# Spimp/sparc_ldpc

Hardware: AMD Instinct MI355X
Metric: decoded codewords/sec (T AMP iters) at L=512,M=512; achieved HBM GB/s vs roofline (higher is better)
Workload: dtype f32; 1 GPU; BASELINE configs[1]: L=512 M=512 R=1 P=4, T=64, single codeword; L=512, M=512, n=4608, T=64, backend=hadamard, precision=fp32, early_stop=False, parallelism=reps sharded over 1 GPU(s)

## Files before the change

### include/sparc_amp.h

```cpp
#ifndef SPARC_AMP_H
#define SPARC_AMP_H

#include <stdint.h>

#ifdef __cplusplus
extern "C" {
#endif

typedef struct sa_ctx sa_ctx;

enum {
  SA_OK = 0,
  SA_ERR_ARG = -1,
  SA_ERR_HIP = -2,
  SA_ERR_NOMEM = -3,
  SA_ERR_ORDERING = -4,
  SA_ERR_UNSUPPORTED = -5,
  SA_ERR_NO_DEVICE = -6
};

enum {
  SA_BACKEND_HADAMARD = 0,
  SA_BACKEND_DENSE = 1,
  SA_BACKEND_HOST = 2,
  SA_BACKEND_MATRIX = 3
};

enum { SA_PREC_F32 = 0, SA_PREC_F64 = 1 };

enum {
  SA_FLAG_NO_EARLY_STOP = 1,
  SA_FLAG_BETA0 = 0x100,
  SA_PTR_DEVICE = 0x200
};

int sa_create(sa_ctx** out, int L, int M, int n, const uint32_t* ordering,
              int backend, int precision, int device);

enum {
  SA_PLAN_DEFAULT = 0,
  SA_PLAN_SEC3 = 1 << 0,
  SA_PLAN_NO_SEC3 = 1 << 1,
  SA_PLAN_ROW16 = 1 << 2,
  SA_PLAN_NO_ROW16 = 1 << 3,
  SA_PLAN_NO_PT = 1 << 4,
  SA_PLAN_ZIL = 1 << 5,
  SA_PLAN_NO_ZIL = 1 << 6,
  SA_PLAN_WB8 = 1 << 7,
  SA_PLAN_WB16 = 1 << 8,
  SA_PLAN_NO_BANKS = 1 << 9,
  SA_PLAN_EAGER = 1 << 10,
  SA_PLAN_ONE_PASS = 1 << 11,
  SA_PLAN_NO_LANES = 1 << 12,
  SA_PLAN_ALL = (1 << 13) - 1
};
int sa_create_ex(sa_ctx** out, int L, int M, int n, const uint32_t* ordering,
                 int backend, int precision, int device, int plan);

int sa_create_matrix(sa_ctx** out, int L, int M, int n, const double* A,
                     int precision, int device);

int sa_create_matrix_random(sa_ctx** out, int L, int M, int n, uint64_t seed, double scale,
                            int precision, int device);

int sa_subset(const sa_ctx* parent, const int64_t* sections, int Ls, sa_ctx** out);

int sa_create_twin(sa_ctx* src, sa_ctx** out);

void sa_destroy(sa_ctx* ctx);

int sa_Ab(sa_ctx* ctx, int B, const double* beta, double* out);

int sa_Az(sa_ctx* ctx, int B, const double* z, double* out);

int sa_amp(sa_ctx* ctx, int B, const double* y, const double* Pl, int T,
           const double* beta0, double* beta_out, int* iters_out, int flags);

int sa_reserve(sa_ctx* ctx, int B, int T);
int sa_stage(sa_ctx* ctx, int B, const double* y, const double* Pl, const double* beta0);
int sa_stage_power_batch(sa_ctx* ctx, int B, const double* Pl);
int sa_run(sa_ctx* ctx, int B, int T, int flags);
int sa_wait(sa_ctx* ctx);
int sa_fetch(sa_ctx* ctx, int B, double* beta_out, int* iters_out);
int sa_fetch_z(sa_ctx* ctx, int B, double* z_out);
int sa_fetch_y(sa_ctx* ctx, int B, double* y_out);
double sa_run_event_ms(sa_ctx* ctx);

// ... 23 lines not shown
                   int32_t* idx_out);

int sa_threshold(sa_ctx* ctx, int B, int l0, int ns, const double* app, int flags, double threshold,
                 int32_t* idx_out);

int sa_cancel(sa_ctx* ctx, int B, const int32_t* idx, sa_ctx* dst);

int sa_cancel_scaled(sa_ctx* ctx, int B, const int32_t* idx, double scale, sa_ctx* dst);

int sa_host_init(sa_ctx* ctx, int B, int T, const double* y, const double* Pl, const double* beta0,
                 const double* ab0);
int sa_host_tau(sa_ctx* ctx, int B, int t, int flags, int* stopped);
int sa_host_eta(sa_ctx* ctx, int B, int t, int flags, const double* az);
int sa_host_residual(sa_ctx* ctx, int B, int t, int flags, const double* ab);

int sa_draw_reps(const uint32_t* seeds, int count, int L, int M, int n, double sigma, int32_t* idx_out,
                 double* noise_out, int threads);
int sa_mc_stage(sa_ctx* ctx, int nreps, const int32_t* idx, const double* noise);
int sa_mc_run(sa_ctx* ctx, int B, int T, int flags, int32_t* dec_out, int32_t* iters_out, int32_t* errs_out,
              double* ms_out);
int sa_mc_draw(sa_ctx* ctx, int nreps, const uint32_t* seeds, const double* sigma, double* ms_out);
int sa_mc_fetch_draws(sa_ctx* ctx, int nreps, int32_t* idx_out, double* noise_out);
int sa_make_ordering(int L, int M, int n, uint32_t seed, uint32_t* out);

typedef enum sa_sec_path {
  SA_SEC_K_SEC = 0,
  SA_SEC_K_SEC2 = 1,
  SA_SEC_K_SECB = 2,
  SA_SEC_DENSE = 3,
  SA_SEC_K_SEC4 = 4,
  SA_SEC_K_SEC43 = 5,
  SA_SEC_DENSE_I8 = 6,
  SA_SEC_MATRIX = 7,
  SA_SEC_K_SECG = 8
} sa_sec_path;
typedef enum sa_row_kernel {
  SA_ROW_K_ROW = 0,
  SA_ROW_K_ROW2 = 1,
  SA_ROW_K_ROWV16 = 2,
  SA_ROW_K_ROWV8 = 3,
  SA_ROW_K_ROW2_16 = 4,
  SA_ROW_K_ROWC = 5
} sa_row_kernel;
int sa_plan(sa_ctx* ctx, int B, int64_t* out8);
int sa_plan_batched(sa_ctx* ctx, int B, int64_t* out4);
int sa_info(const sa_ctx* ctx, int64_t* out8);
int sa_device_count(void);
const char* sa_last_error(void);
const char* sa_version(void);

#ifdef __cplusplus
}
#endif
#endif
```

### sparc_ldpc_amd/_lib.py

```python
from __future__ import annotations

import ctypes as ct
import os

import numpy as np

LIB_NAME = "libsparc_amp.so"
LIB_PATH = os.environ.get("SPARC_AMP_LIB") or os.path.join(os.path.dirname(os.path.abspath(__file__)), LIB_NAME)

SA_OK = 0
SA_ERR_ARG = -1
SA_ERR_HIP = -2
SA_ERR_NOMEM = -3
SA_ERR_ORDERING = -4
SA_ERR_UNSUPPORTED = -5
SA_ERR_NO_DEVICE = -6

SA_BACKEND_HADAMARD = 0
SA_BACKEND_DENSE = 1
SA_BACKEND_HOST = 2
SA_BACKEND_MATRIX = 3
SA_PREC_F32 = 0
SA_PREC_F64 = 1
SA_FLAG_NO_EARLY_STOP = 1
SA_FLAG_BETA0 = 0x100
SA_PTR_DEVICE = 0x200

SA_PLAN = {
    "SEC3": 1 << 0, "NO_SEC3": 1 << 1, "ROW16": 1 << 2, "NO_ROW16": 1 << 3, "NO_PT": 1 << 4,
    "ZIL": 1 << 5, "NO_ZIL": 1 << 6, "WB8": 1 << 7, "WB16": 1 << 8, "NO_BANKS": 1 << 9, "EAGER": 1 << 10,
    "ONE_PASS": 1 << 11, "NO_LANES": 1 << 12,
}


def plan_bits(plan) -> int:
    if plan is None:
        return 0
    if isinstance(plan, int):
        return plan
    if isinstance(plan, str):
        plan = [plan]
    bits = 0
    for name in plan:
        key = name.upper()
        if key not in SA_PLAN:
            raise ValueError(f"unknown plan option {name!r}; known: {sorted(SA_PLAN)}")
        bits |= SA_PLAN[key]
    return bits

EXPORTS = (
    "sa_create", "sa_create_ex", "sa_create_matrix", "sa_create_matrix_random", "sa_subset", "sa_create_twin", "sa_destroy", "sa_Ab", "sa_Az", "sa_amp",
    "sa_reserve", "sa_stage", "sa_stage_power_batch", "sa_run", "sa_wait", "sa_fetch", "sa_fetch_z", "sa_fetch_y", "sa_run_event_ms",
    "sa_profile", "sa_profile_rep", "sa_profile_dispatch", "sa_profile_kinds", "sa_decide",
    "sa_decide_async", "sa_decide_collect", "sa_info", "sa_device_count", "sa_last_error", "sa_version",
    "sa_encode", "sa_stage_onehot", "sa_llr", "sa_soft_beta0", "sa_hard_cancel",
    "sa_threshold", "sa_cancel", "sa_plan", "sa_plan_batched", "sa_stage_onehot_scaled", "sa_cancel_scaled",
    "sa_host_init", "sa_host_tau", "sa_host_eta", "sa_host_residual",
    "sa_draw_reps", "sa_mc_stage", "sa_mc_run", "sa_make_ordering", "sa_mc_draw", "sa_mc_fetch_draws",
)

_P = ct.c_void_p
_I = ct.c_int
_D = ct.POINTER(ct.c_double)
_SIG = {
# ... 119 lines not shown
```

### sparc_ldpc_amd/csrc/sa_host.h

```cpp
#pragma once
#include "sa_common.h"

namespace sa {

struct Prof {
  std::vector<std::tuple<int, hipEvent_t, hipEvent_t>> ev;
  int rep = 1;
  bool dispatch = false;
  int kind = 0;
  int begin(hipStream_t s, int k) {
    kind = k;
    if (dispatch) return 0;
    hipEvent_t a = nullptr, b = nullptr;
    if (add(&a, &b)) return -1;
    return hipEventRecord(a, s) == hipSuccess ? 0 : -1;
  }
  void end(hipStream_t s) {
    if (!dispatch) (void)hipEventRecord(std::get<2>(ev.back()), s);
  }
  int add(hipEvent_t* a, hipEvent_t* b) {
    *a = *b = nullptr;
    if (hipEventCreate(a) != hipSuccess || hipEventCreate(b) != hipSuccess) return -1;
    ev.emplace_back(kind, *a, *b);
    return 0;
// ... 25 lines not shown
  unsigned long long y_ver = 0;
  bool y_read = false;
};

struct sa_ctx {
  sa::Prof* prof = nullptr;
  enum { kLanes = 2 };
  sa_lane lane[kLanes];
  int cur = 0;
  sa_lane& at() { return lane[cur]; }
  const sa_lane& at() const { return lane[cur]; }
  bool lanes_on = false;
  unsigned long long y_ver = 0;
  int y_lane = 0;
  std::vector<double> h_Pl;
  std::vector<double> h_Plb;
  int L = 0, M = 0, n = 0, w = 0, nhi = 0, backend = 0, prec = 0, device = 0;
  int plan = 0;
  bool pow2 = true;
  int Mu = 0, dead = 0;
  int G = 0, NZ = 0, E = 1;
  int n_cus = 256;
  int Gb = 0, CB = 0;
  int WB = 8;
  int gpx = 1 << 20;
  size_t secb_lds = 0;
  int RS = 1, KS = 1, Gd = 0;
  size_t lda = 0;
  size_t sec_lds = 0;
  int G2 = 0;
  int G3 = 0;
  bool sec3 = false;
  size_t sec3_lds = 0;
  uint32_t* d_fwd3 = nullptr;
  bool pt_on = false;
  bool sec4 = false;
  size_t sec4_lds = 0;
  int NZ16 = 0;
  int NZh = 0;
  bool row16 = false;
  int NZ4 = 0, NZ2 = 0;
  bool zil_last = false;
  size_t sec2_lds = 0;
  std::vector<uint32_t> ordering;
  uint16_t* d_inv = nullptr;
  bool big = false;
  uint32_t* d_inv32 = nullptr;
  uint16_t* d_invb = nullptr;
  uint16_t* d_fwdb = nullptr;
  uint16_t* d_invl = nullptr;
  uint32_t* d_hs = nullptr;
  bool borrowed = false;
  bool invb_done = false;
  uint16_t* d_fwd = nullptr;
  uint32_t* d_fwd2 = nullptr;
  void* d_A = nullptr;
  int8_t *d_A8 = nullptr, *d_AT8 = nullptr, *d_zq = nullptr, *d_bq = nullptr;
  double *d_zsc = nullptr, *d_bsc0 = nullptr, *d_bfix = nullptr;
  long long np8 = 0, LMp8 = 0;
  int Bp8 = 0;
  long long np = 0, nk = 0, LMy = 0;
  void *d_AT = nullptr, *d_xz = nullptr, *d_xb = nullptr;
  int fg_cap = 0;
  double cmax = 0;
  int Bcap = 0, Tcap = 0;
  void *d_out = nullptr, *d_c = nullptr, *d_azp = nullptr;
// ... 62 lines not shown
  return SA_OK;
}

constexpr int kI8MinB = 4;
constexpr int kI8MaxS = 16;
constexpr int kFMinB = 4;
constexpr int kFMaxS = 16;

inline size_t rsz(const sa_ctx* c) { return c->prec == SA_PREC_F64 ? 8 : 4; }

inline bool is_dense(const sa_ctx* c) { return c->backend == SA_BACKEND_DENSE || c->backend == SA_BACKEND_MATRIX; }
inline bool use_i8(const sa_ctx* c, int B) { return c->backend == SA_BACKEND_DENSE && B >= kI8MinB; }
inline bool use_fgemm(const sa_ctx* c, int B) { return c->backend == SA_BACKEND_MATRIX && B >= kFMinB; }
inline bool use_batched(const sa_ctx* c, int B) { return c->CB > 0 && B >= 4; }

inline bool zil_for(const sa_ctx* c, int B) {
  const bool on = (c->plan & SA_PLAN_NO_ZIL) ? false : true;
  return on && c->backend == SA_BACKEND_HADAMARD && use_batched(c, B) && c->CB * (int)rsz(c) == 16;
}

int dense_parts(const sa_ctx* c, int B);

struct Plan {
  sa_sec_path sec = SA_SEC_K_SEC;
  sa_row_kernel row = SA_ROW_K_ROW;
  int nz = 0;
  int G = 0, Gb = 0;
  int pt = 0;
  int rs = 1;
  int CB = 1;
  bool zil = false;
  bool dense() const { return sec == SA_SEC_DENSE || sec == SA_SEC_DENSE_I8 || sec == SA_SEC_MATRIX; }
  bool batched() const { return sec == SA_SEC_K_SECB; }
  bool multiwave() const { return sec == SA_SEC_K_SEC2 || sec == SA_SEC_K_SEC4 || sec == SA_SEC_K_SEC43; }
  bool row_sets_iters() const { return row == SA_ROW_K_ROW2 || row == SA_ROW_K_ROW2_16; }
  bool it_row() const { return !dense() && !batched() && row_sets_iters(); }
  bool bzero() const { return sec == SA_SEC_K_SEC4 || sec == SA_SEC_K_SEC43; }
};

inline Plan plan_for(const sa_ctx* c, int B) {
  Plan p;
  const bool f32 = c->prec == SA_PREC_F32;
  p.zil = zil_for(c, B);
  if (p.zil) {
    p.row = SA_ROW_K_ROWC; p.nz = c->NZ2;
  } else if ((long long)B * c->NZ < 4LL * c->n_cus) {
    if (c->row16 && B == 1) { p.row = SA_ROW_K_ROW2_16; p.nz = c->NZh; }
    else { p.row = SA_ROW_K_ROW2; p.nz = c->NZ16; }
  } else if (c->n % (f32 ? 4 : 2) == 0 && (long long)B * (f32 ? c->NZ4 : c->NZ2) >= 2LL * c->n_cus) {
    p.row = SA_ROW_K_ROWV16; p.nz = f32 ? c->NZ4 : c->NZ2;
  } else if (f32 && c->n % 2 == 0 && (long long)B * c->NZ2 >= 2LL * c->n_cus) {
    p.row = SA_ROW_K_ROWV8; p.nz = c->NZ2;
  } else {
    p.row = SA_ROW_K_ROW; p.nz = c->NZ;
  }
  const int wgs = c->G * B;
  p.rs = std::min(4, std::max(1, (c->n_cus + wgs - 1) / wgs));
  if (is_dense(c)) {
    p.sec = use_i8(c, B) ? SA_SEC_DENSE_I8 : (use_fgemm(c, B) ? SA_SEC_MATRIX : SA_SEC_DENSE);
    p.G = dense_parts(c, B);
    p.Gb = c->Gd;
  } else if (use_batched(c, B)) {
    p.sec = SA_SEC_K_SECB;
    p.G = p.Gb = c->Gb;
    p.CB = c->CB;
  } else if (c->backend == SA_BACKEND_HADAMARD && c->G2 > 0 && c->G2 * B * 2 >= c->n_cus) {
    p.sec = c->sec3 ? SA_SEC_K_SEC43 : (c->sec4 ? SA_SEC_K_SEC4 : SA_SEC_K_SEC2);
    p.G = p.Gb = c->sec3 ? c->G3 : c->G2;
    if (p.sec != SA_SEC_K_SEC2 && p.row_sets_iters() && c->pt_on) p.pt = p.row == SA_ROW_K_ROW2_16 ? 16 : kRow2Rows;
  } else {
    p.sec = c->big ? SA_SEC_K_SECG : SA_SEC_K_SEC;
    p.G = p.Gb = c->G;
  }
  return p;
}

template <typename real>
SecArgs<real> sec_args(sa_ctx* c, const Plan& p, int mode, int t, int early_stop, const int* tb = nullptr) {
  SecArgs<real> a;
  const sa_lane& ln = c->at();
  a.inv = c->d_inv; a.inv32 = c->d_inv32; a.invb = c->d_invb; a.invl = c->d_invl; a.hs = c->d_hs;
  a.fwd = (const ushort4*)c->d_fwd;
  a.fwdb = (const ushort4*)c->d_fwdb; a.fwd2 = c->d_fwd2; a.fwd3 = c->d_fwd3; a.c = (const real*)c->d_c;
  a.z = (const real*)ln.d_z; a.beta = (real*)ln.d_beta; a.beta_out = (real*)ln.d_beta; a.out = (real*)c->d_out;
  a.abp = (real*)ln.d_abp; a.bbp = (real*)ln.d_bbp; a.zzp = (const real*)ln.d_zzp;
  a.tau = (real*)ln.d_tau; a.iters = ln.d_iters;
  a.L = c->L; a.M = c->M; a.n = c->n; a.w = c->w; a.nhi = c->nhi; a.G = c->G; a.NZ = p.nz;
  a.T1 = c->Tcap + 1; a.t = t; a.mode = mode; a.early_stop = early_stop;
  a.RS = 1;
  a.pt = 0;
  a.B = 0; a.NC = 0; a.zil = 0; a.gpx = 1 << 20;
  a.cst = c->pb_on ? c->L : 0;
  if (c->pb_on) a.c = (const real*)c->d_cb;
  a.sqrt_n = (real)std::sqrt((double)c->n);
  a.tb = tb;
  a.dead = c->dead;
  a.bzero = 0;
  return a;
}

template <typename real>
// ... 107 lines not shown
```

### sparc_ldpc_amd/csrc/sa_row.hip

```cpp
#include "sa_host.h"

namespace sa {

template <typename real, int kRowWaves>
__global__ void __launch_bounds__(kRowWaves * 64) k_row(RowArgs<real> a) {
  __shared__ real red[kRowWaves][kRowsPerBlk];
  const int b = blockIdx.y, tid = threadIdx.x, lane = tid & 63, wv = tid >> 6;
  const int r = blockIdx.x * kRowsPerBlk + lane;
  const int n = a.n;
  real tau = 1, last = 0;
  if (a.mode == ROW_AMP) {
    tau = ld_vmem(a.tau + (size_t)b * a.T1 + a.t);
    last = a.t > 0 ? ld_vmem(a.tau + (size_t)b * a.T1 + a.t - 1) : (real)0;
  }
  const size_t o = (size_t)b * n + (r < n ? r : 0);
  real yv = 0, zv = 0, Pv = 0, bbv[2] = {0, 0};
  if (wv == 0) {
    yv = a.y[o];
    if (a.mode == ROW_AMP) {
      zv = a.z[o];
      Pv = ld_vmem(a.Pb + (size_t)b * a.Pbst);
      const real* bp = a.bbp + (size_t)b * a.Gb;
      bbv[0] = lane < a.Gb ? bp[lane] : (real)0;
      bbv[1] = lane + 64 < a.Gb ? bp[lane + 64] : (real)0;
// ... 272 lines not shown
  const int rl = tid & (R - 1), pg = tid / R;
  const int r = blockIdx.x * R + rl;
  real tau = 1, last = 0;
  if (mode == ROW_AMP) {
    tau = ld_vmem(tau_p + (size_t)b * T1 + t);
    last = t > 0 ? ld_vmem(tau_p + (size_t)b * T1 + t - 1) : (real)0;
  }
  const size_t o = (size_t)b * n + (r < n ? r : 0);
  real yv = 0, zv = 0, Pv = 0, bbv[4] = {0, 0, 0, 0};
  if (tid < 64) {
    yv = y_p[o];
    if (mode == ROW_AMP) {
      zv = zin_p[o];
      Pv = ld_vmem(Pb_p + (size_t)b * Pbst);
      const real* bp = bbp_p + (size_t)b * Gb;
#pragma unroll
      for (int q = 0; q < 4; ++q) bbv[q] = tid + 64 * q < Gb ? bp[tid + 64 * q] : (real)0;
    }
  }
  if (mode != ROW_INIT0) {
    const size_t gs = pt ? (size_t)R : (size_t)n;
    const real* p = pt ? abp_p + (size_t)b * G * ((size_t)NZ * R) + (size_t)blockIdx.x * G * R + rl
                       : abp_p + (size_t)b * G * n + (r < n ? r : 0);
    real acc = 0;
    constexpr int U = 256 / NG;
    if (pt && (R == 16 || sizeof(real) == 4) && G == NG * U) {
      const real* pb = abp_p + (size_t)b * G * ((size_t)NZ * R) + (size_t)blockIdx.x * G * R;
      real tt[U];
#pragma unroll
      for (int u = 0; u < U; ++u)
        tt[u] = ld_off(pb, (unsigned)(((pg + NG * u) * R + rl) * (int)sizeof(real)));
#pragma unroll
      for (int u = 0; u < U; ++u) acc += tt[u];
    } else
    for (int g0 = pg; g0 < G; g0 += NG * U) {
      real tt[U];
#pragma unroll
      for (int u = 0; u < U; ++u) {
        const int g = g0 + NG * u;
        tt[u] = p[(size_t)(g < G ? g : pg) * gs];
      }
#pragma unroll
      for (int u = 0; u < U; ++u)
        if (g0 + NG * u < G) acc += tt[u];
    }
    red[pg][rl] = acc;
  }
  if (mode == ROW_AMP && es && tau == last) return;
  const real tau2 = tau * tau;
  __syncthreads();
  if (tid >= 64) return;
  if (itset != 0 && blockIdx.x == 0 && tid == 0) iters_p[b] = itset;
  real ons = 0;
  if (mode == ROW_AMP) {
    real bb;
    if (Gb <= 256) {
      real sacc = 0;
#pragma unroll
      for (int q = 0; q < 4; ++q) sacc += bbv[q];
      bb = wave_sum(sacc);
    } else {
      bb = wave_sum_parts(bbp_p + (size_t)b * Gb, Gb);
    }
    ons = Pv - bb / (real)n;
  }
  real zn = 0;
// ... 90 lines not shown
```

### sparc_ldpc_amd/csrc/sa_sec.hip

```cpp
#include "sa_host.h"

namespace sa {



template <typename real, int E>
__global__ void __launch_bounds__(256) k_sec(SecArgs<real> a) {
  STAMP(0);
  extern __shared__ __attribute__((aligned(16))) unsigned char smem[];
  constexpr int KH = E >= 16 ? 2 : (E >= 8 ? 16 : 16);
  constexpr int NQ = (E + 3) / 4;
  constexpr int KR = 8;
  int g, rsi;
  if (a.RS > 1 && (a.G & 7) == 0) {
    const int j = blockIdx.x, u = j >> 3;
    rsi = u % a.RS;
    g = (u / a.RS) * 8 + (j & 7);
  } else {
    g = blockIdx.x / a.RS;
    rsi = blockIdx.x % a.RS;
  }
  const int b = blockIdx.y;
  const int rows_per = (a.n + a.RS - 1) / a.RS;
  const int rb0 = rsi * rows_per, rb1 = min(a.n, rb0 + rows_per);
// ... 450 lines not shown
  for (int i = 0; i < EQ; ++i) xs[q * QS + i * 64 + lane] = v[i];
  __syncthreads();
#pragma unroll
  for (int i = 0; i < EQ; ++i) {
    real x[QW];
#pragma unroll
    for (int j = 0; j < QW; ++j) x[j] = xs[j * QS + i * 64 + lane];
#pragma unroll
    for (int k = 0, span = 1; span < QW; ++k, span <<= 1)
#pragma unroll
      for (int j = 0; j < QW; j += 2 * span) x[j] = ((q >> k) & 1) ? x[j] - x[j + span] : x[j] + x[j + span];
    v[i] = x[0];
  }
  __syncthreads();
}

template <typename real, int QW, bool MAX>
__device__ __forceinline__ real combine_q(const real* red, int w0, int f) {
  real x[QW];
#pragma unroll
  for (int j = 0; j < QW; ++j) x[j] = red[(w0 + j) * 4 + f];
#pragma unroll
  for (int span = 1; span < QW; span <<= 1)
#pragma unroll
    for (int j = 0; j < QW; j += 2 * span) {
      if constexpr (MAX) x[j] = x[j] > x[j + span] ? x[j] : x[j + span];
      else x[j] = x[j] + x[j + span];
    }
  return x[0];
}

template <typename real, int EQ, int QW, int SPW = 2>
__device__ __forceinline__ void secq_body(const SecArgs<real>& a) {
  static_assert(SPW == 2 || SPW == 3, "sections per workgroup");
  STAMP(0);
  extern __shared__ __attribute__((aligned(16))) unsigned char smem[];
  constexpr int NT = SPW * QW * 64;
  constexpr int KH = EQ >= 8 ? 4 : (SPW == 3 ? 8 : 16);
  constexpr int NQ = (EQ + 3) / 4;
  constexpr int KR = ((SPW == 3 ? 8448 : 4608) + NT - 1) / NT;
  const int g = blockIdx.x, b = blockIdx.y;
  const int tid = threadIdx.x, lane = tid & 63, wv = tid >> 6;
  const int sidx = wv / QW, q = wv % QW;
  const int M = a.M, n = a.n, Mq = M / QW;
  const size_t LM = (size_t)a.L * M;
  const int l = g * SPW + sidx;
  const bool have = l < a.L;
  const int lc = have ? l : a.L - 1;
  const int eoff = q * Mq;

  real* zs = reinterpret_cast<real*>(smem);
  const int zslots = ((n + 1) * (int)sizeof(real) + 15) / 16 * 16 / (int)sizeof(real);
  real* ts = zs + zslots;
  real* xb = ts + SPW * M;
  real* red = xb + SPW * M;

  real v[EQ];
  real bprev[EQ];
  const real* bl = a.beta + (size_t)b * LM + (size_t)lc * M + eoff;
  real* blo = a.beta_out + (size_t)b * LM + (size_t)lc * M + eoff;
  const uint16_t* ibase = a.inv + (size_t)g * SPW * a.w;
  const unsigned ioff = (unsigned)((lc - g * SPW) * a.w + eoff);
  const uint32_t* fw = (SPW == 2 ? a.fwd2 : a.fwd3) + (size_t)g * n;
  ushort4 tb[KH][NQ];
  uint32_t f[KR];

  const real* zb = a.z + (size_t)b * n;
  ZStage<real, NT> zst;
  const real* zzb = a.zzp + (size_t)b * a.NZ;
  ZZParts<real, 5> zz;
  const bool dma = stage_z_dma<real, NT>(zb, zs, n, tid);
  if (!dma) zst.issue(zb, n, tid);
  zz.issue(zzb, a.NZ, lane);
  const real last = a.t > 0 ? ld_vmem(a.tau + (size_t)b * a.T1 + a.t - 1) : (real)0;
  load_buckets_off<EQ, KH>(ibase, ioff, 0, a.nhi, M, lane, tb);
  load_section<real, EQ>(bl, bprev, lane, Mq);
  const real cl = ld_vmem(a.c + (size_t)b * a.cst + lc);
  const real tau = zz.tau(zzb, a.NZ, n);
  if (a.bzero) {
#pragma unroll
    for (int i = 0; i < EQ; ++i) bprev[i] = 0;
  }
  const bool stop = a.early_stop && (tau == last);
  if (g == 0 && tid == 0) {
    a.tau[(size_t)b * a.T1 + a.t] = tau;
    if (stop && a.iters[b] < 0) a.iters[b] = a.t;
  }
  if (stop) {
    if (dma) asm volatile("s_waitcnt vmcnt(0)" ::: "memory");
    if (a.bzero && have) {
      store_section<real, EQ>(a.beta + (size_t)b * LM + (size_t)lc * M + eoff, bprev, lane, Mq);
    }
    return;
  }
  const real tau2 = tau * tau;
  const real inv_sn = (real)1 / a.sqrt_n;
  const real kk = cl / tau2;
  STAMP(1);
  if (!dma) zst.store(zs, zb, n, tid);
  else finish_z_dma<real>(zb, zs, n, tid);
  __syncthreads();
  STAMP(2);
#ifdef SA_STAMPS
  asm volatile("s_waitcnt vmcnt(0)" ::: "memory");
  STAMP(10);
#endif
#pragma unroll
  for (int i = 0; i < EQ; ++i) v[i] = 0;
  for (int h0 = 0; h0 < a.nhi; h0 += KH) {
    ushort4 tn[KH][NQ];
    const bool more = h0 + KH < a.nhi;
    if (more) load_buckets_off<EQ, KH>(ibase, ioff, h0 + KH, a.nhi, M, lane, tn);
    gather_buckets<real, EQ, KH>(zs, h0, a.nhi, tb, v);
    if (more) {
#pragma unroll
      for (int hh = 0; hh < KH; ++hh)
#pragma unroll
        for (int j = 0; j < NQ; ++j) tb[hh][j] = tn[hh][j];
    }
  }
  real* xs = xb + sidx * M;
#pragma unroll
  for (int u = 0; u < KR; ++u) {
    const int r = u * NT + tid;
    f[u] = ld_off(fw, (unsigned)(r < n ? r : 0) * 4u);
  }
  STAMP(3);
  fwht_wave<real, EQ>(v, lane, 64);
  topq_stage<real, EQ, QW>(v, xs, lane, q);
  STAMP(4);


  real mx = neg_inf<real>();
#pragma unroll
  for (int i = 0; i < EQ; ++i) {
    v[i] = fma(v[i], inv_sn, bprev[i]) * kk;
    mx = v[i] > mx ? v[i] : mx;
  }
  mx = wave_max(mx);
  if (lane == 0) red[wv * 4] = mx;
  __syncthreads();
  const int w0 = wv & ~(QW - 1);
  mx = combine_q<real, QW, true>(red, w0, 0);
  real S = 0, S2 = 0;
#pragma unroll
  for (int i = 0; i < EQ; ++i) {
    v[i] = dexp<real>(v[i] - mx);
    S += v[i];
    S2 += v[i] * v[i];
  }
  wave_sum2(S, S2);
  if (lane == 0) {
    red[wv * 4 + 1] = S;
    red[wv * 4 + 2] = S2;
  }
  __syncthreads();
  S = combine_q<real, QW, false>(red, w0, 1);
  S2 = combine_q<real, QW, false>(red, w0, 2);
  const real scale = cl * rcp_fast(S);
#pragma unroll
  for (int i = 0; i < EQ; ++i) v[i] = have ? v[i] * scale : (real)0;
  if (have) store_section<real, EQ>(blo, v, lane, Mq);
  const real bb = have ? S2 * scale * scale : (real)0;

  STAMP(5);
  fwht_wave<real, EQ>(v, lane, 64);
  topq_stage<real, EQ, QW>(v, xs, lane, q);
  STAMP(6);
  {
    real* tl = ts + sidx * M + eoff;
#pragma unroll
    for (int i = 0; i < EQ; ++i) tl[elem_index<EQ>(lane, i)] = v[i];
  }
  if (lane == 0) red[wv * 4 + 3] = bb;
  __syncthreads();
  STAMP(7);
  if (tid == 0) {
    real bsum = red[0 * 4 + 3] + red[QW * 4 + 3];
    if constexpr (SPW == 3) bsum += red[2 * QW * 4 + 3];
    a.bbp[(size_t)b * a.G + g] = bsum;
  }
  real* abp = a.abp + ((size_t)b * a.G + g) * n;
  const int psh = a.pt == 16 ? 4 : 5;
  const size_t npad = (size_t)((n + (1 << psh) - 1) >> psh) << psh;
  real* abq = a.abp + (size_t)b * a.G * npad + ((size_t)g << psh);
  real* const sbase = a.pt ? abq : abp;
  const int sh = a.pt ? psh : 31;
  const size_t gstride = (size_t)a.G << sh;
  const int smask = (int)((1u << sh) - 1u);
  static_assert(NT % 32 == 0, "a pass of rows is a whole number of row blocks");
  const size_t ustep = sh < 31 ? (size_t)(NT >> sh) * gstride : (size_t)NT;
  for (int r0 = 0; r0 < n; r0 += NT * KR) {
    if (r0 > 0) {
#pragma unroll
      for (int u = 0; u < KR; ++u) {
        const int r = r0 + u * NT + tid;
        f[u] = fw[r < n ? r : 0];
      }
    }
    real* const pbase = sbase + (size_t)((r0 + tid) >> sh) * gstride + ((r0 + tid) & smask);
    auto row = [&](int u, int r) {
      real t;
      if constexpr (SPW == 2) {
        const uint32_t e = f[u];
        const real v0 = ts[e & 0x7fffu];
        const real v1 = ts[M + ((e >> 16) & 0x7fffu)];
        t = (e & 0x8000u) ? -v0 : v0;
        t += (e & 0x80000000u) ? -v1 : v1;
      } else {
        const uint32_t e = f[u];
        const real v0 = ts[e & 0x1ffu];
        const real v1 = ts[M + ((e >> 10) & 0x1ffu)];
        const real v2 = ts[2 * M + ((e >> 20) & 0x1ffu)];
        t = (e & 0x200u) ? -v0 : v0;
        t += (e & 0x80000u) ? -v1 : v1;
        t += (e & 0x20000000u) ? -v2 : v2;
      }
      if constexpr (SPW == 3) st_part(pbase + u * ustep, t);
      else st_part(&sbase[(size_t)(r >> sh) * gstride + (r & smask)], t);
    };
    if (r0 + NT * KR <= n) {
#pragma unroll
      for (int u = 0; u < KR; ++u) row(u, r0 + u * NT + tid);
    } else {
#pragma unroll
      for (int u = 0; u < KR; ++u) {
        const int r = r0 + u * NT + tid;
        if (r < n) row(u, r);
      }
    }
  }
#ifdef SA_STAMPS
  STAMP(8);
  asm volatile("s_waitcnt vmcnt(0)" ::: "memory");
  STAMP(9);
#endif
}

template <typename real, int E4>
__global__ void __launch_bounds__(512) k_sec4(SecArgs<real> a) { secq_body<real, E4, 4, 2>(a); }
template <typename real, int E4>
__global__ void __launch_bounds__(768) k_sec43(SecArgs<real> a) { secq_body<real, E4, 4, 3>(a); }

template <typename real, int E>
void launch_sec_e(sa_ctx* c, const Plan& p, int B, SecArgs<real> a) {
  a.RS = p.rs;
  dim3 grid(c->G * a.RS, B);
  if (c->prof) c->prof->begin(c->at().stream, K_SEC);
  if (c->big)
    plaunch(c, k_secg<real, E>, grid, 256, c->sec_lds, a);
  else
    plaunch(c, k_sec<real, E>, grid, 256, c->sec_lds, a);
  if (c->prof) c->prof->end(c->at().stream);
}

template <typename real>
int launch_sec2(sa_ctx* c, const Plan& p, int B, int t, int es, void* bin, void* bout, int bzero) {
  SecArgs<real> a = sec_args<real>(c, p, SEC_AMP, t, es);
  a.pt = p.pt;
  if (bzero && !p.bzero()) return fail(SA_ERR_UNSUPPORTED, "k_sec2 reads its previous estimate");
  a.bzero = bzero;
  a.beta = (real*)bin;
  a.beta_out = (real*)bout;
  a.G = p.G;
  dim3 grid(a.G, B);
  if (c->prof) c->prof->begin(c->at().stream, K_SEC);
  switch (p.sec) {
    case SA_SEC_K_SEC43:
      switch (c->M / 256) {
        case 1: plaunch(c, k_sec43<real, 1>, grid, 768, c->sec3_lds, a); break;
        case 2: plaunch(c, k_sec43<real, 2>, grid, 768, c->sec3_lds, a); break;
        default: return fail(SA_ERR_UNSUPPORTED, "k_sec43: M");
      }
      break;
    case SA_SEC_K_SEC4:
      switch (c->M / 256) {
        case 1: plaunch(c, k_sec4<real, 1>, grid, 512, c->sec4_lds, a); break;
        case 2: plaunch(c, k_sec4<real, 2>, grid, 512, c->sec4_lds, a); break;
        case 4: plaunch(c, k_sec4<real, 4>, grid, 512, c->sec4_lds, a); break;
        case 8: plaunch(c, k_sec4<real, 8>, grid, 512, c->sec4_lds, a); break;
        case 16: plaunch(c, k_sec4<real, 16>, grid, 512, c->sec4_lds, a); break;
        default: return fail(SA_ERR_UNSUPPORTED, "k_sec4: M");
      }
      break;
    case SA_SEC_K_SEC2:
      switch (c->M / 128) {
        case 1: plaunch(c, k_sec2<real, 1>, grid, 256, c->sec2_lds, a); break;
        case 2: plaunch(c, k_sec2<real, 2>, grid, 256, c->sec2_lds, a); break;
        case 4: plaunch(c, k_sec2<real, 4>, grid, 256, c->sec2_lds, a); break;
        case 8: plaunch(c, k_sec2<real, 8>, grid, 256, c->sec2_lds, a); break;
        case 16: plaunch(c, k_sec2<real, 16>, grid, 256, c->sec2_lds, a); break;
        case 32: plaunch(c, k_sec2<real, 32>, grid, 256, c->sec2_lds, a); break;
        default: return fail(SA_ERR_UNSUPPORTED, "k_sec2: M");
      }
      break;
    default: return fail(SA_ERR_ARG, "launch_sec2: the plan runs no multi-wave section kernel");
  }
  if (c->prof) c->prof->end(c->at().stream);
  HIP_TRY(hipGetLastError());
  return SA_OK;
}

template <typename real>
int launch_sec(sa_ctx* c, const Plan& p, int B, int mode, int t, int es, void* bin, void* bout) {
  SecArgs<real> a = sec_args<real>(c, p, mode, t, es);
  if (bin) a.beta = (real*)bin;
  if (bout) a.beta_out = (real*)bout;
  switch (c->E) {
    case 1: launch_sec_e<real, 1>(c, p, B, a); break;
    case 2: launch_sec_e<real, 2>(c, p, B, a); break;
    case 4: launch_sec_e<real, 4>(c, p, B, a); break;
    case 8: launch_sec_e<real, 8>(c, p, B, a); break;
    case 16: launch_sec_e<real, 16>(c, p, B, a); break;
    case 32: launch_sec_e<real, 32>(c, p, B, a); break;
    case 64: launch_sec_e<real, 64>(c, p, B, a); break;
    default: return fail(SA_ERR_UNSUPPORTED, "bad E");
  }
  HIP_TRY(hipGetLastError());
  return SA_OK;
}

template int launch_sec<float>(sa_ctx*, const Plan&, int, int, int, int, void*, void*);
template int launch_sec<double>(sa_ctx*, const Plan&, int, int, int, int, void*, void*);
template int launch_sec2<float>(sa_ctx*, const Plan&, int, int, int, void*, void*, int);
template int launch_sec2<double>(sa_ctx*, const Plan&, int, int, int, void*, void*, int);

template <typename real>
static hipError_t sec_lds_attrs_t() {
  const int mx = 160 * 1024;
  hipError_t e = hipSuccess;
#define SA_A(F) if (e == hipSuccess) e = hipFuncSetAttribute((const void*)F, hipFuncAttributeMaxDynamicSharedMemorySize, mx);
  SA_A((k_sec<real, 1>)) SA_A((k_sec<real, 2>)) SA_A((k_sec<real, 4>)) SA_A((k_sec<real, 8>))
  SA_A((k_sec<real, 16>)) SA_A((k_sec<real, 32>)) SA_A((k_sec<real, 64>))
  SA_A((k_secg<real, 1>)) SA_A((k_secg<real, 2>)) SA_A((k_secg<real, 4>)) SA_A((k_secg<real, 8>))
  SA_A((k_secg<real, 16>)) SA_A((k_secg<real, 32>)) SA_A((k_secg<real, 64>))
  SA_A((k_sec2<real, 1>)) SA_A((k_sec2<real, 2>)) SA_A((k_sec2<real, 4>)) SA_A((k_sec2<real, 8>))
  SA_A((k_sec2<real, 16>)) SA_A((k_sec2<real, 32>))
  SA_A((k_sec4<real, 1>)) SA_A((k_sec4<real, 2>)) SA_A((k_sec4<real, 4>)) SA_A((k_sec4<real, 8>))
  SA_A((k_sec4<real, 16>))
  SA_A((k_sec43<real, 1>)) SA_A((k_sec43<real, 2>))
#undef SA_A
  return e;
}

hipError_t sec_lds_attrs() {
  hipError_t e = sec_lds_attrs_t<float>();
  return e == hipSuccess ? sec_lds_attrs_t<double>() : e;
}

#ifdef SA_STAMPS
hipError_t stamps_add_sec(unsigned long long* out) {
  unsigned long long s[16 * 16];
  hipError_t e = hipMemcpyFromSymbol(s, HIP_SYMBOL(g_stamps), sizeof(s));
  for (int i = 0; i < 16 * 16; ++i) out[i] += s[i];
  return e;
}
#endif

}
```

### sparc_ldpc_amd/csrc/sparc_amp.hip

```cpp

#define SA_VERSION "sparc_amp 0.4 gfx950"

#include "sa_host.h"

namespace sa {

thread_local std::string g_err;

int fail(int code, const std::string& msg) {
  g_err = msg;
  return code;
}

template <typename src_t, typename dst_t>
__global__ void k_convert(const src_t* s, dst_t* d, size_t N) {
  for (size_t i = blockIdx.x * (size_t)blockDim.x + threadIdx.x; i < N;
       i += (size_t)gridDim.x * blockDim.x)
    d[i] = (dst_t)s[i];
}

__global__ void k_fill32(uint32_t* p, uint32_t v, size_t nw) {
  for (size_t i = blockIdx.x * (size_t)blockDim.x + threadIdx.x; i < nw; i += (size_t)gridDim.x * blockDim.x)
    p[i] = v;
}
// ... 972 lines not shown
    const auto c8 = nob ? std::pair<int, size_t>{0, 0} : cb_for(kWB);
    const auto c16 = nob ? std::pair<int, size_t>{0, 0} : cb_for(kWB16);
    const bool w16 = (plan & SA_PLAN_WB16) ? true
                     : (plan & SA_PLAN_WB8) ? false
                                            : c16.first >= c8.first;
    c->WB = w16 && c16.first > 0 ? kWB16 : kWB;
    c->CB = c->WB == kWB16 ? c16.first : c8.first;
    c->secb_lds = c->WB == kWB16 ? c16.second : c8.second;
    c->Gb = (L + c->WB - 1) / c->WB;
    const size_t per_group = (size_t)c->WB * ((size_t)c->w + (size_t)n) * 2;
    const int gx = c->Gb / 8 > 0 ? c->Gb / 8 : 1;
    const int fit = (int)std::max<size_t>(1, kSecbL2 / per_group);
    int npass = (gx + fit - 1) / fit;
    c->gpx = (gx + npass - 1) / npass;
    if (plan & SA_PLAN_ONE_PASS) c->gpx = 1 << 20;
  }
  {
    hipDeviceProp_t prop;
    if (hipGetDeviceProperties(&prop, device) == hipSuccess && prop.multiProcessorCount > 0)
      c->n_cus = prop.multiProcessorCount;
  }
  c->Gd = (L + 3) / 4;
  {
    const size_t need3 = (((size_t)(n + 1) * s + 15) / 16 * 16) + 6 * (size_t)M * s + 48 * s;
    const int G3 = (L + 2) / 3;
    const bool fits = c->sec4 && backend == SA_BACKEND_HADAMARD && M <= 512 && need3 <= 160 * 1024;
    const bool over = c->G2 > c->n_cus || (s == 8 && c->G2 == c->n_cus);
    const bool want = (plan & SA_PLAN_SEC3) ? true : (plan & SA_PLAN_NO_SEC3) ? false : (over && G3 <= c->n_cus);
    if (fits && want) {
      c->sec3 = true;
      c->G3 = G3;
      c->sec3_lds = need3;
    }
  }
  if (lane_open(c->lane[0]) != SA_OK) {
    delete c;
    return fail(SA_ERR_HIP, "stream/event creation failed");
  }
  int rc = SA_OK;
  if (backend == SA_BACKEND_DENSE) {
    c->RS = 8;
    c->KS = 8;
    rc = build_tables(c);
    if (!rc) rc = build_dense(c);
  } else if (backend == SA_BACKEND_HOST) {
    c->lda = (size_t)L * M;
  } else if (backend == SA_BACKEND_MATRIX) {
    c->RS = 8;
    c->KS = 8;
    rc = matrix_init(c);
  } else if (share) {
    c->d_inv = share->d_inv; c->d_inv32 = share->d_inv32; c->d_invb = share->d_invb;
    c->d_fwdb = share->d_fwdb; c->d_fwd = share->d_fwd; c->d_fwd2 = share->d_fwd2; c->d_fwd3 = share->d_fwd3;
    c->d_invl = share->d_invl; c->d_hs = share->d_hs;
    c->invb_done = share->invb_done;
    c->borrowed = true;
  } else {
    rc = build_tables(c);
  }
  if (!rc) rc = dev_alloc(c, &c->d_c, (size_t)L * s);
  if (!rc) rc = dev_alloc(c, (void**)&c->d_cd, (size_t)L * 8);
  if (!rc) rc = dev_alloc(c, &c->d_P1, s);
  if (rc) {
    sa_destroy(c);
    return rc;
  }
// ... 420 lines not shown
```

### sparc_ldpc_amd/operators.py

```python
from __future__ import annotations

import hashlib
import os
from collections import OrderedDict

import numpy as np

from . import _lib
from ._lib import as_f64, check, dptr

__all__ = [
    "SparcOperator", "AbOp", "AzOp", "HostOperatorLoop", "make_ordering", "sub_fht", "block_sub_fht",
    "sparc_transforms", "sparc_transforms_shorter", "dense_transforms", "gaussian_transforms", "default_device",
]

_BACKENDS = {"hadamard": _lib.SA_BACKEND_HADAMARD, "dense": _lib.SA_BACKEND_DENSE}
_PRECS = {"fp32": _lib.SA_PREC_F32, "fp64": _lib.SA_PREC_F64}

DEFAULT_BACKEND = os.environ.get("SPARC_AMP_BACKEND", "hadamard")
DEFAULT_PRECISION = os.environ.get("SPARC_AMP_PRECISION", "fp32")


def default_device() -> int:
    lib = _lib.load()
# ... 202 lines not shown
        check(self._lib.sa_wait(self._ctx))

    def last_run_ms(self) -> float:
        return float(self._lib.sa_run_event_ms(self._ctx))

    KERNEL_KINDS = ("k_sec", "k_row", "k_dense_az", "k_dense_den", "k_dense_ab", "k_i8_quant")

    def profile(self, B, T, early_stop=True, beta0=False, rep=1):
        flags = (0 if early_stop else _lib.SA_FLAG_NO_EARLY_STOP) | (_lib.SA_FLAG_BETA0 if beta0 else 0)
        nk = len(self.KERNEL_KINDS)
        if int(self._lib.sa_profile_kinds()) != nk:
            raise _lib.SparcAmpError(_lib.SA_ERR_UNSUPPORTED, f"libsparc_amp profiles {self._lib.sa_profile_kinds()} kernel kinds, "
                                f"this module knows {nk}: rebuild the library")
        out = np.zeros(2 * nk + 1)
        if rep == 0:
            check(self._lib.sa_profile_dispatch(self._ctx, int(B), int(T), flags, dptr(out)))
        else:
            check(self._lib.sa_profile_rep(self._ctx, int(B), int(T), flags, int(rep), dptr(out)))
        kinds = {k: (float(out[2 * i]), int(out[2 * i + 1])) for i, k in enumerate(self.KERNEL_KINDS)}
        return kinds, float(out[2 * nk])

    def fetch(self, B):
        out = np.empty((B, self.L * self.M))
        iters = np.empty(B, dtype=np.int32)
        check(self._lib.sa_fetch(self._ctx, B, dptr(out), iters.ctypes.data_as(_lib.ct.POINTER(_lib.ct.c_int))))
        return out, iters

    def iters(self, B):
        it = np.empty(B, dtype=np.int32)
        check(self._lib.sa_fetch(self._ctx, B, None, it.ctypes.data_as(_lib.ct.POINTER(_lib.ct.c_int))))
        return it

    SECTION_KERNELS = ("k_sec", "k_sec2", "k_secb", "dense", "k_sec4", "k_sec43", "dense_mfma", "matrix_mfma",
                       "k_secg")
    ROW_KERNELS = ("k_row", "k_row2", "k_rowv16B", "k_rowv8B", "k_row2_16", "k_rowc")

    def fetch_z(self, B):
        z = np.empty((B, self.n))
        check(self._lib.sa_fetch_z(self._ctx, int(B), z.ctypes.data_as(_lib.ct.POINTER(_lib.ct.c_double))))
        return z

    def fetch_y(self, B):
        y = np.empty((B, self.n))
        check(self._lib.sa_fetch_y(self._ctx, int(B), dptr(y)))
        return y

    def plan(self, B):
        o = np.zeros(8, dtype=np.int64)
        check(self._lib.sa_plan(self._ctx, int(B), o.ctypes.data_as(_lib.ct.POINTER(_lib.ct.c_int64))))
        return dict(section_kernel=self.SECTION_KERNELS[int(o[0])], partials=int(o[1]), row_splits=int(o[2]),
                    codewords_per_wg=int(o[3]), zz_partials=int(o[4]), w=int(o[5]),
                    row_kernel=self.ROW_KERNELS[int(o[6])], cus=int(o[7]))

    def mc_supported(self, B):
        if self.backend != "hadamard" or not 4 <= int(B) <= 1024:
            return False
        p = self.plan(B)
        return p["section_kernel"] == "k_secb" and p["row_kernel"] == "k_rowc"

    def mc_stage(self, idx, noise):
        idx = np.ascontiguousarray(idx, dtype=np.int32)
        R = idx.shape[0]
        assert idx.shape == (R, self.L), "idx must be (R, L)"
        noise = as_f64(noise)
        assert noise.size == R * self.n, "noise must be (R, n)"
        check(self._lib.sa_mc_stage(self._ctx, R, idx.ctypes.data_as(_lib.ct.POINTER(_lib.ct.c_int32)), dptr(noise)))
        self._mc_reps = R
# ... 316 lines not shown
```

Before: 2275 codewords/s.

## Add opt-in four-sections-per-workgroup section kernel and adjust row16 default

```diff
diff --git a/include/sparc_amp.h b/include/sparc_amp.h
--- a/include/sparc_amp.h
+++ b/include/sparc_amp.h
@@ -52,7 +52,9 @@
   SA_PLAN_EAGER = 1 << 10,
   SA_PLAN_ONE_PASS = 1 << 11,
   SA_PLAN_NO_LANES = 1 << 12,
-  SA_PLAN_ALL = (1 << 13) - 1
+  SA_PLAN_SEC4Q = 1 << 13,
+  SA_PLAN_NO_SEC4Q = 1 << 14,
+  SA_PLAN_ALL = (1 << 15) - 1
 };
 int sa_create_ex(sa_ctx** out, int L, int M, int n, const uint32_t* ordering,
                  int backend, int precision, int device, int plan);
@@ -142,7 +144,8 @@
   SA_SEC_K_SEC43 = 5,
   SA_SEC_DENSE_I8 = 6,
   SA_SEC_MATRIX = 7,
-  SA_SEC_K_SECG = 8
+  SA_SEC_K_SECG = 8,
+  SA_SEC_K_SEC44 = 9
 } sa_sec_path;
 typedef enum sa_row_kernel {
   SA_ROW_K_ROW = 0,
diff --git a/sparc_ldpc_amd/_lib.py b/sparc_ldpc_amd/_lib.py
--- a/sparc_ldpc_amd/_lib.py
+++ b/sparc_ldpc_amd/_lib.py
@@ -29,7 +29,7 @@
 SA_PLAN = {
     "SEC3": 1 << 0, "NO_SEC3": 1 << 1, "ROW16": 1 << 2, "NO_ROW16": 1 << 3, "NO_PT": 1 << 4,
     "ZIL": 1 << 5, "NO_ZIL": 1 << 6, "WB8": 1 << 7, "WB16": 1 << 8, "NO_BANKS": 1 << 9, "EAGER": 1 << 10,
-    "ONE_PASS": 1 << 11, "NO_LANES": 1 << 12,
+    "ONE_PASS": 1 << 11, "NO_LANES": 1 << 12, "SEC4Q": 1 << 13, "NO_SEC4Q": 1 << 14,
 }
 
 
diff --git a/sparc_ldpc_amd/csrc/sa_host.h b/sparc_ldpc_amd/csrc/sa_host.h
--- a/sparc_ldpc_amd/csrc/sa_host.h
+++ b/sparc_ldpc_amd/csrc/sa_host.h
@@ -81,6 +81,9 @@
   int G3 = 0;
   bool sec3 = false;
   size_t sec3_lds = 0;
+  int G4 = 0;
+  bool sec4q = false;
+  size_t sec4q_lds = 0;
   uint32_t* d_fwd3 = nullptr;
   bool pt_on = false;
   bool sec4 = false;
@@ -209,10 +212,12 @@
   bool zil = false;
   bool dense() const { return sec == SA_SEC_DENSE || sec == SA_SEC_DENSE_I8 || sec == SA_SEC_MATRIX; }
   bool batched() const { return sec == SA_SEC_K_SECB; }
-  bool multiwave() const { return sec == SA_SEC_K_SEC2 || sec == SA_SEC_K_SEC4 || sec == SA_SEC_K_SEC43; }
+  bool multiwave() const {
+    return sec == SA_SEC_K_SEC2 || sec == SA_SEC_K_SEC4 || sec == SA_SEC_K_SEC43 || sec == SA_SEC_K_SEC44;
+  }
   bool row_sets_iters() const { return row == SA_ROW_K_ROW2 || row == SA_ROW_K_ROW2_16; }
   bool it_row() const { return !dense() && !batched() && row_sets_iters(); }
-  bool bzero() const { return sec == SA_SEC_K_SEC4 || sec == SA_SEC_K_SEC43; }
+  bool bzero() const { return sec == SA_SEC_K_SEC4 || sec == SA_SEC_K_SEC43 || sec == SA_SEC_K_SEC44; }
 };
 
 inline Plan plan_for(const sa_ctx* c, int B) {
@@ -242,8 +247,8 @@
     p.G = p.Gb = c->Gb;
     p.CB = c->CB;
   } else if (c->backend == SA_BACKEND_HADAMARD && c->G2 > 0 && c->G2 * B * 2 >= c->n_cus) {
-    p.sec = c->sec3 ? SA_SEC_K_SEC43 : (c->sec4 ? SA_SEC_K_SEC4 : SA_SEC_K_SEC2);
-    p.G = p.Gb = c->sec3 ? c->G3 : c->G2;
+    p.sec = c->sec3 ? SA_SEC_K_SEC43 : (c->sec4q ? SA_SEC_K_SEC44 : (c->sec4 ? SA_SEC_K_SEC4 : SA_SEC_K_SEC2));
+    p.G = p.Gb = c->sec3 ? c->G3 : (c->sec4q ? c->G4 : c->G2);
     if (p.sec != SA_SEC_K_SEC2 && p.row_sets_iters() && c->pt_on) p.pt = p.row == SA_ROW_K_ROW2_16 ? 16 : kRow2Rows;
   } else {
     p.sec = c->big ? SA_SEC_K_SECG : SA_SEC_K_SEC;
diff --git a/sparc_ldpc_amd/csrc/sa_row.hip b/sparc_ldpc_amd/csrc/sa_row.hip
--- a/sparc_ldpc_amd/csrc/sa_row.hip
+++ b/sparc_ldpc_amd/csrc/sa_row.hip
@@ -328,6 +328,15 @@
         tt[u] = ld_off(pb, (unsigned)(((pg + NG * u) * R + rl) * (int)sizeof(real)));
 #pragma unroll
       for (int u = 0; u < U; ++u) acc += tt[u];
+    } else if (pt && (R == 16 || sizeof(real) == 4) && G == NG * (U / 2)) {
+      constexpr int UH = U / 2;
+      const real* pb = abp_p + (size_t)b * G * ((size_t)NZ * R) + (size_t)blockIdx.x * G * R;
+      real tt[UH];
+#pragma unroll
+      for (int u = 0; u < UH; ++u)
+        tt[u] = ld_off(pb, (unsigned)(((pg + NG * u) * R + rl) * (int)sizeof(real)));
+#pragma unroll
+      for (int u = 0; u < UH; ++u) acc += tt[u];
     } else
     for (int g0 = pg; g0 < G; g0 += NG * U) {
       real tt[U];
diff --git a/sparc_ldpc_amd/csrc/sa_sec.hip b/sparc_ldpc_amd/csrc/sa_sec.hip
--- a/sparc_ldpc_amd/csrc/sa_sec.hip
+++ b/sparc_ldpc_amd/csrc/sa_sec.hip
@@ -506,13 +506,14 @@
 
 template <typename real, int EQ, int QW, int SPW = 2>
 __device__ __forceinline__ void secq_body(const SecArgs<real>& a) {
-  static_assert(SPW == 2 || SPW == 3, "sections per workgroup");
+  static_assert(SPW == 2 || SPW == 3 || SPW == 4, "sections per workgroup");
   STAMP(0);
   extern __shared__ __attribute__((aligned(16))) unsigned char smem[];
   constexpr int NT = SPW * QW * 64;
-  constexpr int KH = EQ >= 8 ? 4 : (SPW == 3 ? 8 : 16);
+  constexpr int KH = EQ >= 8 ? 4 : ((SPW == 3 || (SPW == 4 && sizeof(real) == 8)) ? 8 : 16);
   constexpr int NQ = (EQ + 3) / 4;
   constexpr int KR = ((SPW == 3 ? 8448 : 4608) + NT - 1) / NT;
+  constexpr int FW = SPW == 4 ? 2 : 1;
   const int g = blockIdx.x, b = blockIdx.y;
   const int tid = threadIdx.x, lane = tid & 63, wv = tid >> 6;
   const int sidx = wv / QW, q = wv % QW;
@@ -535,9 +536,10 @@
   real* blo = a.beta_out + (size_t)b * LM + (size_t)lc * M + eoff;
   const uint16_t* ibase = a.inv + (size_t)g * SPW * a.w;
   const unsigned ioff = (unsigned)((lc - g * SPW) * a.w + eoff);
-  const uint32_t* fw = (SPW == 2 ? a.fwd2 : a.fwd3) + (size_t)g * n;
+  const uint32_t* fw = (SPW == 3 ? a.fwd3 : a.fwd2) + (size_t)(SPW == 4 ? 2 * g : g) * n;
+  const uint32_t* fw1 = a.fwd2 + (size_t)(2 * g + 1 < (a.L + 1) / 2 ? 2 * g + 1 : 2 * g) * n;
   ushort4 tb[KH][NQ];
-  uint32_t f[KR];
+  uint32_t f[KR][FW];
 
   const real* zb = a.z + (size_t)b * n;
   ZStage<real, NT> zst;
@@ -597,7 +599,8 @@
 #pragma unroll
   for (int u = 0; u < KR; ++u) {
     const int r = u * NT + tid;
-    f[u] = ld_off(fw, (unsigned)(r < n ? r : 0) * 4u);
+    f[u][0] = ld_off(fw, (unsigned)(r < n ? r : 0) * 4u);
+    if constexpr (SPW == 4) f[u][1] = ld_off(fw1, (unsigned)(r < n ? r : 0) * 4u);
   }
   STAMP(3);
   fwht_wave<real, EQ>(v, lane, 64);
@@ -651,7 +654,8 @@
   STAMP(7);
   if (tid == 0) {
     real bsum = red[0 * 4 + 3] + red[QW * 4 + 3];
-    if constexpr (SPW == 3) bsum += red[2 * QW * 4 + 3];
+    if constexpr (SPW >= 3) bsum += red[2 * QW * 4 + 3];
+    if constexpr (SPW == 4) bsum += red[3 * QW * 4 + 3];
     a.bbp[(size_t)b * a.G + g] = bsum;
   }
   real* abp = a.abp + ((size_t)b * a.G + g) * n;
@@ -669,20 +673,32 @@
 #pragma unroll
       for (int u = 0; u < KR; ++u) {
         const int r = r0 + u * NT + tid;
-        f[u] = fw[r < n ? r : 0];
+        f[u][0] = fw[r < n ? r : 0];
+        if constexpr (SPW == 4) f[u][1] = fw1[r < n ? r : 0];
       }
     }
     real* const pbase = sbase + (size_t)((r0 + tid) >> sh) * gstride + ((r0 + tid) & smask);
     auto row = [&](int u, int r) {
       real t;
       if constexpr (SPW == 2) {
-        const uint32_t e = f[u];
+        const uint32_t e = f[u][0];
         const real v0 = ts[e & 0x7fffu];
         const real v1 = ts[M + ((e >> 16) & 0x7fffu)];
         t = (e & 0x8000u) ? -v0 : v0;
         t += (e & 0x80000000u) ? -v1 : v1;
+      } else if constexpr (SPW == 4) {
+        const uint32_t e = f[u][0], e1 = f[u][1];
+        const real v0 = ts[e & 0x7fffu];
+        const real v1 = ts[M + ((e >> 16) & 0x7fffu)];
+        const real v2 = ts[2 * M + (e1 & 0x7fffu)];
+        const real v3 = ts[3 * M + ((e1 >> 16) & 0x7fffu)];
+        t = (e & 0x8000u) ? -v0 : v0;
+        t += (e & 0x80000000u) ? -v1 : v1;
+        real t1 = (e1 & 0x8000u) ? -v2 : v2;
+        t1 += (e1 & 0x80000000u) ? -v3 : v3;
+        t += t1;
       } else {
-        const uint32_t e = f[u];
+        const uint32_t e = f[u][0];
         const real v0 = ts[e & 0x1ffu];
         const real v1 = ts[M + ((e >> 10) & 0x1ffu)];
         const real v2 = ts[2 * M + ((e >> 20) & 0x1ffu)];
@@ -696,6 +712,10 @@
     if (r0 + NT * KR <= n) {
 #pragma unroll
       for (int u = 0; u < KR; ++u) row(u, r0 + u * NT + tid);
+    } else if (SPW == 4 && r0 + NT * (KR - 1) <= n) {
+#pragma unroll
+      for (int u = 0; u < KR - 1; ++u) row(u, r0 + u * NT + tid);
+      if (r0 + (KR - 1) * NT + tid < n) row(KR - 1, r0 + (KR - 1) * NT + tid);
     } else {
 #pragma unroll
       for (int u = 0; u < KR; ++u) {
@@ -715,6 +735,8 @@
 __global__ void __launch_bounds__(512) k_sec4(SecArgs<real> a) { secq_body<real, E4, 4, 2>(a); }
 template <typename real, int E4>
 __global__ void __launch_bounds__(768) k_sec43(SecArgs<real> a) { secq_body<real, E4, 4, 3>(a); }
+template <typename real, int E4>
+__global__ void __launch_bounds__(1024) k_sec44(SecArgs<real> a) { secq_body<real, E4, 4, 4>(a); }
 
 template <typename real, int E>
 void launch_sec_e(sa_ctx* c, const Plan& p, int B, SecArgs<real> a) {
@@ -747,6 +769,13 @@
         default: return fail(SA_ERR_UNSUPPORTED, "k_sec43: M");
       }
       break;
+    case SA_SEC_K_SEC44:
+      switch (c->M / 256) {
+        case 1: plaunch(c, k_sec44<real, 1>, grid, 1024, c->sec4q_lds, a); break;
+        case 2: plaunch(c, k_sec44<real, 2>, grid, 1024, c->sec4q_lds, a); break;
+        default: return fail(SA_ERR_UNSUPPORTED, "k_sec44: M");
+      }
+      break;
     case SA_SEC_K_SEC4:
       switch (c->M / 256) {
         case 1: plaunch(c, k_sec4<real, 1>, grid, 512, c->sec4_lds, a); break;
@@ -813,6 +842,7 @@
   SA_A((k_sec4<real, 1>)) SA_A((k_sec4<real, 2>)) SA_A((k_sec4<real, 4>)) SA_A((k_sec4<real, 8>))
   SA_A((k_sec4<real, 16>))
   SA_A((k_sec43<real, 1>)) SA_A((k_sec43<real, 2>))
+  SA_A((k_sec44<real, 1>)) SA_A((k_sec44<real, 2>))
 #undef SA_A
   return e;
 }
diff --git a/sparc_ldpc_amd/csrc/sparc_amp.hip b/sparc_ldpc_amd/csrc/sparc_amp.hip
--- a/sparc_ldpc_amd/csrc/sparc_amp.hip
+++ b/sparc_ldpc_amd/csrc/sparc_amp.hip
@@ -1028,6 +1028,15 @@
       c->G3 = G3;
       c->sec3_lds = need3;
     }
+    const size_t need4q = zbytes + 8 * (size_t)M * s + 64 * s;
+    const bool fits4q = c->sec4 && backend == SA_BACKEND_HADAMARD && M <= 512 && need4q <= 160 * 1024;
+    if (fits4q && (plan & SA_PLAN_SEC4Q) && !(plan & (SA_PLAN_SEC3 | SA_PLAN_NO_SEC4Q))) {
+      c->sec4q = true;
+      c->sec3 = false;
+      c->G4 = (L + 3) / 4;
+      c->sec4q_lds = need4q;
+    }
+    if (c->G2 == c->n_cus && !(plan & (SA_PLAN_ROW16 | SA_PLAN_NO_SEC3))) c->row16 = false;
   }
   if (lane_open(c->lane[0]) != SA_OK) {
     delete c;
diff --git a/sparc_ldpc_amd/operators.py b/sparc_ldpc_amd/operators.py
--- a/sparc_ldpc_amd/operators.py
+++ b/sparc_ldpc_amd/operators.py
@@ -258,7 +258,7 @@
         return it
 
     SECTION_KERNELS = ("k_sec", "k_sec2", "k_secb", "dense", "k_sec4", "k_sec43", "dense_mfma", "matrix_mfma",
-                       "k_secg")
+                       "k_secg", "k_sec44")
     ROW_KERNELS = ("k_row", "k_row2", "k_rowv16B", "k_rowv8B", "k_row2_16", "k_rowc")
 
     def fetch_z(self, B):
```

Measured after the change: 2347 codewords/s, median of 6. +3.1%, better.
